# montyhall/bot7

Hardware: AMD Instinct MI355X
Metric: EI candidates scored/sec at N=2048,d=32 (higher is better)
Workload: dtype f64

## Files before the change

### bot7_amd/build.py

```python
import concurrent.futures
import os
import subprocess
import sys

HERE = os.path.dirname(os.path.abspath(__file__))
ROOT = os.path.dirname(HERE)
CSRC = os.path.join(HERE, "csrc")
BUILD = os.path.join(HERE, "_build")
OUT = os.path.join(HERE, "libbot7hip.so")
SOURCES = ["context.hip", "grid_api.hip", "gp_api.hip", "nominate.hip", "blr_api.hip", "sobol.hip", "covar.hip", "potrf.hip", "potrf_persist.hip", "posterior.hip", "score.hip", "extras.hip", "comm.hip", "group.hip", "blr_small.hip", "gp_small.hip", "kpost_small.hip", "batch.hip", "mes.hip", "rff.hip", "slice.hip", "refine.hip", "kg.hip"]
DIAG_ONLY_SOURCES = ["nll_small.hip"]
DIAG_OUT = os.path.join(ROOT, "tools", "_build", "libbot7hip_diag.so")
HEADERS = [os.path.join(CSRC, "b7_internal.h"), os.path.join(CSRC, "gemm_f64.h"), os.path.join(CSRC, "potrf_diag.h"), os.path.join(CSRC, "comm_rccl.h"), os.path.join(CSRC, "ksx_exp.h"), os.path.join(CSRC, "exp_table.h"), os.path.join(CSRC, "mes_math.h"), os.path.join(CSRC, "counter_rng.h"), os.path.join(CSRC, "gp_small_body.h"),
           os.path.join(ROOT, "include", "bot7hip.h")]
HIPCC = os.environ.get("HIPCC", "/opt/rocm/bin/hipcc")
FLAGS = ["-O3", "-std=c++17", "-fPIC", "--offload-arch=gfx950", "-fno-fast-math", "-Wall",
         "-I" + os.path.join(ROOT, "include"), "-I" + CSRC, "-I/opt/rocm/include"]


def _stale(target, deps):
    if not os.path.exists(target):
        return True
    t = os.path.getmtime(target)
    return any(os.path.getmtime(d) > t for d in deps)


EXTRA_FLAGS = {"covar.hip": ["-mllvm", "-amdgpu-mfma-vgpr-form"], "batch.hip": ["-mllvm", "-amdgpu-mfma-vgpr-form"],
               "rff.hip": ["-mllvm", "-amdgpu-mfma-vgpr-form"],
               "kg.hip": ["-mllvm", "-amdgpu-mfma-vgpr-form"],
               "slice.hip": ["-mllvm", "-disable-machine-licm"]}


def _compile(src, diag=False):
    obj = os.path.join(BUILD, ("diag_" if diag else "") + src.replace(".hip", ".o"))
    path = os.path.join(CSRC, src)
    if _stale(obj, [path] + HEADERS + [os.path.abspath(__file__)]):
        subprocess.check_call([HIPCC] + FLAGS + EXTRA_FLAGS.get(src, []) + (["-DB7_DIAG"] if diag else []) + ["-c", path, "-o", obj])
        return obj, True
    return obj, False


def _mentions_diag(src):
    return "B7_DIAG" in open(os.path.join(CSRC, src)).read()


def build_diag(verbose=False):
    build()
    os.makedirs(os.path.dirname(DIAG_OUT), exist_ok=True)
    todo = [s for s in SOURCES if _mentions_diag(s)] + DIAG_ONLY_SOURCES
    with concurrent.futures.ThreadPoolExecutor(max_workers=min(8, len(todo))) as ex:
        res = dict(zip(todo, ex.map(lambda s: _compile(s, True), todo)))
    objs = [res[s][0] if s in res else os.path.join(BUILD, s.replace(".hip", ".o")) for s in SOURCES + DIAG_ONLY_SOURCES]
    if any(ch for _, ch in res.values()) or _stale(DIAG_OUT, objs):
        subprocess.check_call([HIPCC, "-shared", "-fPIC", "--offload-arch=gfx950", "-o", DIAG_OUT] + objs +
                              ["-ldl", "-Wl,-rpath,/opt/rocm/lib", "-Wl,--no-undefined", "-Wl,-Bsymbolic"])
        if verbose:
            print("built", DIAG_OUT)
    return DIAG_OUT


def posterior_isa():
    out = os.path.join(BUILD, "posterior.s")
    path = os.path.join(CSRC, "posterior.hip")
    if _stale(out, [path] + HEADERS + [os.path.abspath(__file__)]):
        subprocess.check_call([HIPCC] + [f for f in FLAGS if f != "-fPIC"] + ["-S", "--cuda-device-only", "-Wno-unused-command-line-argument",
                                                                            path, "-o", out])
    return out


def check_agpr_discipline():
    import re
    text = open(posterior_isa()).read()
    found = {}
    for m in re.finditer(r"^(_ZN\S*post_kernel_w4(?:ILi(\d)E|tILi\d+ELi\d+E)\S*):[^\n]*\n(.*?)\n\s*s_endpgm", text, flags=re.S | re.M):
        nj = int(m.group(2)) if m.group(2) else 16
        ntiles = 32 if nj == 16 else 8 * nj
        in_asm, stats, bad = False, {"mfma": 0, "mfma_from_zero": 0, "acc_reads": 0, "scratch": 0}, []
        for line in m.group(3).split("\n"):
            code = line.split(";")[0]
            if "ASMSTART" in line:
                in_asm = True
                continue
            if "ASMEND" in line:
                in_asm = False
                continue
            if in_asm:
                stats["mfma"] += "v_mfma_f64_16x16x4_f64" in code
                stats["mfma_from_zero"] += bool(re.search(r"v_mfma_f64_16x16x4_f64 a\[[^\]]*\], v\[[^\]]*\], v\[[^\]]*\], 0\s*$", code))
                stats["acc_reads"] += "v_accvgpr_read_b32" in code
            else:
                if re.search(r"(?<![A-Za-z0-9_.])a(\[|\d)", code):
                    bad.append(line.strip())
                stats["scratch"] += "scratch_" in code
        if bad or stats["scratch"] or stats["mfma_from_zero"] != ntiles or stats["acc_reads"] != 8 * ntiles:
            raise RuntimeError("post_kernel_w4<%d>: AGPR discipline broken: %r, compiler-generated AGPR uses: %r"
                               % (nj, stats, bad[:5]))
        found[nj] = stats
    if not {2, 4} <= set(found):
        raise RuntimeError("post_kernel_w4<2> and <4> expected in the ISA of posterior.hip, found %r" % sorted(found))
    return found


def build_post_probe():
    src = os.path.join(ROOT, "tools", "post_probe.hip")
    out = os.path.join(ROOT, "tools", "_build", "post_probe")
    os.makedirs(os.path.dirname(out), exist_ok=True)
    if _stale(out, [src, os.path.join(ROOT, "tools", "post_kernel_w8.h"), os.path.join(CSRC, "posterior.hip")] + HEADERS):
        subprocess.check_call([HIPCC, "--offload-arch=gfx950", "-O3", "-std=c++17", "-fno-fast-math", "-Wno-unused-value",
                               "-DB7_POST_NO_LAUNCHERS", "-I" + os.path.join(ROOT, "include"), "-I" + CSRC,
                               "-I/opt/rocm/include", "-o", out, src, "-Wl,-rpath,/opt/rocm/lib"])
    return out


def build(force=False, verbose=False):
    os.makedirs(BUILD, exist_ok=True)
    if force:
        for f in os.listdir(BUILD):
            os.remove(os.path.join(BUILD, f))
    with concurrent.futures.ThreadPoolExecutor(max_workers=min(8, len(SOURCES) + 2)) as ex:
        isa = ex.submit(check_agpr_discipline)
        probe = ex.submit(build_post_probe)
        results = list(ex.map(_compile, SOURCES))
        isa.result()
        probe.result()
    objs = [o for o, _ in results]
    if any(changed for _, changed in results) or _stale(OUT, objs):
        subprocess.check_call([HIPCC, "-shared", "-fPIC", "--offload-arch=gfx950", "-o", OUT] + objs +
                              ["-ldl", "-Wl,-rpath,/opt/rocm/lib", "-Wl,--no-undefined", "-Wl,-Bsymbolic"])
        if verbose:
            print("built", OUT)
    return OUT


if __name__ == "__main__":
    build(force="--force" in sys.argv, verbose=True)
    if "--diag" in sys.argv:
        build_diag(verbose=True)
```

### bot7_amd/csrc/posterior.hip

```cpp
#include "b7_internal.h"
#include <utility>

#ifdef B7_POST_STAMPS
__device__ unsigned long long b7_post_stamps[4 * 4096];
extern "C" int b7dbg_post_stamps(unsigned long long *out, int nblocks) {
  return (int)hipMemcpyFromSymbol(out, HIP_SYMBOL(b7_post_stamps), sizeof(unsigned long long) * 4 * nblocks);
}
#endif

typedef double d2_t __attribute__((ext_vector_type(2)));

struct PostBatch {
  int64_t sLinv = 0, sks = 0, svar = 0;
  const double *base = nullptr, *var_add = nullptr;
};

namespace w4 {
constexpr int BM = 128, BK = 16, LD = BK + 1, A_DBL = BM * LD;

#define B7_W4_ACC_REGS \
  "a0", "a1", "a2", "a3", "a4", "a5", "a6", "a7", "a8", "a9", "a10", "a11", "a12", "a13", "a14", "a15", \
  "a16", "a17", "a18", "a19", "a20", "a21", "a22", "a23", "a24", "a25", "a26", "a27", "a28", "a29", "a30", \
  "a31", "a32", "a33", "a34", "a35", "a36", "a37", "a38", "a39", "a40", "a41", "a42", "a43", "a44", "a45", \
  "a46", "a47", "a48", "a49", "a50", "a51", "a52", "a53", "a54", "a55", "a56", "a57", "a58", "a59", "a60", \
  "a61", "a62", "a63", "a64", "a65", "a66", "a67", "a68", "a69", "a70", "a71", "a72", "a73", "a74", "a75", \
  "a76", "a77", "a78", "a79", "a80", "a81", "a82", "a83", "a84", "a85", "a86", "a87", "a88", "a89", "a90", \
  "a91", "a92", "a93", "a94", "a95", "a96", "a97", "a98", "a99", "a100", "a101", "a102", "a103", "a104", \
  "a105", "a106", "a107", "a108", "a109", "a110", "a111", "a112", "a113", "a114", "a115", "a116", "a117", \
  "a118", "a119", "a120", "a121", "a122", "a123", "a124", "a125", "a126", "a127", "a128", "a129", "a130", \
  "a131", "a132", "a133", "a134", "a135", "a136", "a137", "a138", "a139", "a140", "a141", "a142", "a143", \
  "a144", "a145", "a146", "a147", "a148", "a149", "a150", "a151", "a152", "a153", "a154", "a155", "a156", \
  "a157", "a158", "a159", "a160", "a161", "a162", "a163", "a164", "a165", "a166", "a167", "a168", "a169", \
  "a170", "a171", "a172", "a173", "a174", "a175", "a176", "a177", "a178", "a179", "a180", "a181", "a182", \
  "a183", "a184", "a185", "a186", "a187", "a188", "a189", "a190", "a191", "a192", "a193", "a194", "a195", \
  "a196", "a197", "a198", "a199", "a200", "a201", "a202", "a203", "a204", "a205", "a206", "a207", "a208", \
  "a209", "a210", "a211", "a212", "a213", "a214", "a215", "a216", "a217", "a218", "a219", "a220", "a221", \
  "a222", "a223", "a224", "a225", "a226", "a227", "a228", "a229", "a230", "a231", "a232", "a233", "a234", \
  "a235", "a236", "a237", "a238", "a239", "a240", "a241", "a242", "a243", "a244", "a245", "a246", "a247", \
  "a248", "a249", "a250", "a251", "a252", "a253", "a254", "a255"

template <int NJ, int I, int J, bool ZERO>
__device__ __forceinline__ void mfma_tile(double a, double b) {
  constexpr int lo = 8 * (NJ * I + J);
  if constexpr (ZERO)
    asm volatile("v_mfma_f64_16x16x4_f64 a[%2:%3], %0, %1, 0" ::"v"(a), "v"(b), "n"(lo), "n"(lo + 7) : B7_W4_ACC_REGS);
  else
    asm volatile("v_mfma_f64_16x16x4_f64 a[%2:%3], %0, %1, a[%2:%3]" ::"v"(a), "v"(b), "n"(lo), "n"(lo + 7)
                 : B7_W4_ACC_REGS);
}

template <int NJ, int I, int J>
__device__ __forceinline__ void read_tile(double (&v)[4]) {
  constexpr int lo = 8 * (NJ * I + J);
  unsigned w[8];
  asm volatile(
      "v_accvgpr_read_b32 %0, a[%8]\n\tv_accvgpr_read_b32 %1, a[%9]\n\tv_accvgpr_read_b32 %2, a[%10]\n\t"
      "v_accvgpr_read_b32 %3, a[%11]\n\tv_accvgpr_read_b32 %4, a[%12]\n\tv_accvgpr_read_b32 %5, a[%13]\n\t"
      "v_accvgpr_read_b32 %6, a[%14]\n\tv_accvgpr_read_b32 %7, a[%15]"
      : "=v"(w[0]), "=v"(w[1]), "=v"(w[2]), "=v"(w[3]), "=v"(w[4]), "=v"(w[5]), "=v"(w[6]), "=v"(w[7])
      : "n"(lo), "n"(lo + 1), "n"(lo + 2), "n"(lo + 3), "n"(lo + 4), "n"(lo + 5), "n"(lo + 6), "n"(lo + 7));
#pragma unroll
  for (int r = 0; r < 4; ++r) v[r] = __hiloint2double((int)w[2 * r + 1], (int)w[2 * r]);
}

template <int NJ>
struct Frags {
  double a[2][8], b[2][NJ];
};
template <int NJ>
struct Stage {
  d2_t c[4 + 2 * NJ];
};
struct Cursor {
  int t, kb, ntiles;
  __device__ __forceinline__ void advance() {
    if (kb + 1 < (t + 1) * (BM / BK)) {
      ++kb;
    } else if (t + 1 < ntiles) {
      ++t;
      kb = 0;
    }
  }
};

template <int N, class F, int... Is>
__device__ __forceinline__ void static_for_impl(F &&f, std::integer_sequence<int, Is...>) {
  (f(std::integral_constant<int, Is>{}), ...);
}
template <int N, class F>
__device__ __forceinline__ void static_for(F &&f) {
  static_for_impl<N>(f, std::make_integer_sequence<int, N>{});
}

template <int NJ, int P, int S0>
__device__ __forceinline__ void read_pair(Frags<NJ> &f, const double *__restrict__ sa, const double *__restrict__ sb) {
  if constexpr (P < NJ) {
    f.b[0][P] = sb[P * 16 * LD + 4 * S0];
    f.b[1][P] = sb[P * 16 * LD + 4 * S0 + 4];
  } else {
    f.a[0][P - NJ] = sa[(P - NJ) * 16 * LD + 4 * S0];
    f.a[1][P - NJ] = sa[(P - NJ) * 16 * LD + 4 * S0 + 4];
  }
}

template <int NJ, int C>
__device__ __forceinline__ void load_chunk(Stage<NJ> &g, const double *__restrict__ qa, const double *__restrict__ qb,
                                           int64_t lda) {
  if constexpr (C < 4)
    g.c[C] = *reinterpret_cast<const d2_t *>(qa + (int64_t)(32 * C) * lda);
  else
    g.c[C] = *reinterpret_cast<const d2_t *>(qb + (int64_t)(32 * (C - 4)) * lda);
}
template <int NJ, int C>
__device__ __forceinline__ void store_chunk(const Stage<NJ> &g, double *__restrict__ w) {
  constexpr int o = C < 4 ? 32 * C * LD : A_DBL + 32 * (C - 4) * LD;
  w[o] = g.c[C][0];
  w[o + 1] = g.c[C][1];
}

template <int NJ, int FIRST, bool ZERO>
__device__ __forceinline__ void stage(Frags<NJ> &f0, Frags<NJ> &f1, Stage<NJ> &g, double *__restrict__ cur,
                                      double *__restrict__ nxt, int fa, int fb, int wofs, const double *__restrict__ pa,
                                      const double *__restrict__ pb, int64_t lda, Cursor &ld) {
  constexpr int NI = 8 - FIRST, NM = 2 * NJ * NI, NP = 8 + NJ, NC = 4 + 2 * NJ, NS = NP + 2 * NC;
  const double *qa = pa + ((int64_t)ld.t * BM) * lda + ld.kb * BK, *qb = pb + ld.kb * BK;
  ld.advance();
  constexpr int K1 = (NS + NM - 1) / NM + 1, K2 = (NP + NM - 1) / NM + 1;
  static_for<NM>([&](auto m_) {
    constexpr int m = decltype(m_)::value, ks = m / (NJ * NI), i = FIRST + (m % (NJ * NI)) / NJ, j = m % NJ;
    mfma_tile<NJ, i, j, ZERO && ks == 0>(f0.a[ks][i], f0.b[ks][j]);
    static_for<K1>([&](auto k_) {
      constexpr int sidx = m * NS / NM + decltype(k_)::value;
      if constexpr (sidx < (m + 1) * NS / NM) {
        if constexpr (sidx < NP) {
          if constexpr (sidx < NJ || sidx - NJ >= FIRST) read_pair<NJ, sidx, 2>(f1, cur + fa, cur + fb);
        } else if constexpr (sidx < NP + NC) {
          store_chunk<NJ, sidx - NP>(g, nxt + wofs);
        } else {
          load_chunk<NJ, sidx - NP - NC>(g, qa, qb, lda);
        }
      }
    });
  });
  __builtin_amdgcn_s_waitcnt(0xC07F);
  __builtin_amdgcn_s_barrier();
  static_for<NM>([&](auto m_) {
    constexpr int m = decltype(m_)::value, ks = m / (NJ * NI), i = FIRST + (m % (NJ * NI)) / NJ, j = m % NJ;
    mfma_tile<NJ, i, j, false>(f1.a[ks][i], f1.b[ks][j]);
    static_for<K2>([&](auto k_) {
      constexpr int sidx = m * NP / NM + decltype(k_)::value;
      if constexpr (sidx < (m + 1) * NP / NM) read_pair<NJ, sidx, 0>(f0, nxt + fa, nxt + fb);
    });
  });
}

template <int NJ>
__global__ void __launch_bounds__(256)
    post_kernel_w4(const double *__restrict__ Linv, const double *__restrict__ ks, int Npad, int64_t row0, int64_t Mtotal,
                   double base, double sgn, double var_add, int clamp, double var_min, double *__restrict__ var,
                   PostBatch bat) {
  constexpr int BN = 64 * NJ, STAGE_DBL = (BM + BN) * LD, NC = 4 + 2 * NJ, NP = 8 + NJ;
  extern __shared__ __align__(16) double sm[];
  if (bat.base) {
    const int64_t y = blockIdx.y;
    Linv += y * bat.sLinv;
    ks += y * bat.sks;
    var += y * bat.svar;
    base = bat.base[y];
    if (bat.var_add) var_add = bat.var_add[y];
  }
  const int lane = threadIdx.x & 63, wave = __builtin_amdgcn_readfirstlane(threadIdx.x >> 6);
#ifdef B7_POST_STAMPS
  const unsigned long long st0 = __builtin_amdgcn_s_memtime(), sr0 = __builtin_amdgcn_s_memrealtime();
  __builtin_amdgcn_s_waitcnt(0xC07F);
#endif
  const int64_t lda = Npad;
  const int r0 = threadIdx.x >> 3, kc = threadIdx.x & 7;
  const double *pa = Linv + (int64_t)r0 * lda + 2 * kc;
  const double *pb = ks + ((int64_t)blockIdx.x * BN + r0) * lda + 2 * kc;
  const int wofs = r0 * LD + 2 * kc;
  const int fa = (lane & 15) * LD + (lane >> 4);
  const int fb = A_DBL + (wave * 16 * NJ + (lane & 15)) * LD + (lane >> 4);

  const int ntiles = Npad / BM;
  Cursor ld{0, 0, ntiles};
  Stage<NJ> g;
  Frags<NJ> f0, f1;
  double *const b0 = sm, *const b1 = sm + STAGE_DBL;
  static_for<NC>([&](auto c_) { load_chunk<NJ, decltype(c_)::value>(g, pa, pb, lda); });
  ld.advance();
  static_for<NC>([&](auto c_) { store_chunk<NJ, decltype(c_)::value>(g, b0 + wofs); });
  {
    const double *qa = pa + ((int64_t)ld.t * BM) * lda + ld.kb * BK, *qb = pb + ld.kb * BK;
    static_for<NC>([&](auto c_) { load_chunk<NJ, decltype(c_)::value>(g, qa, qb, lda); });
    ld.advance();
  }
  __builtin_amdgcn_s_waitcnt(0xC07F);
  __builtin_amdgcn_s_barrier();
  static_for<NP>([&](auto p_) { read_pair<NJ, decltype(p_)::value, 0>(f0, b0 + fa, b0 + fb); });

  double colss[2][NJ] = {};
#define B7_STAGE(F, Z, CUR, NXT) stage<NJ, F, Z>(f0, f1, g, CUR, NXT, fa, fb, wofs, pa, pb, lda, ld)
  for (int t = 0; t < ntiles; ++t) {
    B7_STAGE(0, true, b0, b1);
    if (t > 0) {
      for (int p = 0; p < 4 * t - 1; ++p) {
        B7_STAGE(0, false, b1, b0);
        B7_STAGE(0, false, b0, b1);
      }
      B7_STAGE(0, false, b1, b0);
      B7_STAGE(0, false, b0, b1);
    }
    B7_STAGE(1, false, b1, b0);
    B7_STAGE(2, false, b0, b1);
    B7_STAGE(3, false, b1, b0);
    B7_STAGE(4, false, b0, b1);
    B7_STAGE(5, false, b1, b0);
    B7_STAGE(6, false, b0, b1);
    B7_STAGE(7, false, b1, b0);
    asm volatile("s_nop 15\n\ts_nop 15\n\ts_nop 15" ::: "memory");
    static_for<2 * NJ>([&](auto hj_) {
      constexpr int h = decltype(hj_)::value / NJ, j = decltype(hj_)::value % NJ;
      double s = 0.0;
      static_for<4>([&](auto i_) {
        double v[4];
        read_tile<NJ, 4 * h + decltype(i_)::value, j>(v);
#pragma unroll
        for (int r = 0; r < 4; ++r) s = __builtin_fma(v[r], v[r], s);
      });
      colss[h][j] += s;
    });
  }
#undef B7_STAGE

#pragma unroll
  for (int j = 0; j < NJ; ++j) {
    double v0 = colss[0][j], v1 = colss[1][j];
    v0 += __shfl_xor(v0, 16);
    v0 += __shfl_xor(v0, 32);
    v1 += __shfl_xor(v1, 16);
    v1 += __shfl_xor(v1, 32);
    const int64_t gidx = row0 + (int64_t)blockIdx.x * BN + wave * 16 * NJ + j * 16 + lane;
    if (lane < 16 && gidx < Mtotal) {
      double ss = v0;
      ss += v1;
      double v = (base + sgn * ss) + var_add;
      if (clamp) v = (v < var_min) ? var_min : v;
      var[gidx] = v;
    }
  }
#ifdef B7_POST_STAMPS
  if (threadIdx.x == 0 && blockIdx.x < 4096) {
    const unsigned long long st1 = __builtin_amdgcn_s_memtime(), sr1 = __builtin_amdgcn_s_memrealtime();
    __builtin_amdgcn_s_waitcnt(0xC07F);
    unsigned long long *o = b7_post_stamps + 4 * blockIdx.x;
    o[0] = st0, o[1] = sr0, o[2] = st1, o[3] = sr1;
  }
#endif
}

template <int NJ>
constexpr int lds_bytes() { return 2 * (BM + 64 * NJ) * LD * 8; }

template <int NJ, int NR>
struct Tall {
  static constexpr int BMT = 16 * NR, BN = 64 * NJ, A_DBLT = BMT * LD, STAGE_DBL = (BMT + BN) * LD;
  static constexpr int NCA = BMT / 32, NC = NCA + 2 * NJ, NP = NR + NJ;
  static constexpr int LDS_BYTES = 2 * STAGE_DBL * 8;
  static_assert(NJ * NR == 32, "32 accumulator tiles per wave");

  struct Set {
    double a[NR], b[NJ];
  };
  struct Data {
    d2_t c[NC];
  };
  struct Cursor {
    int t, kb, ntiles;
    __device__ __forceinline__ void advance() {
      if (kb + 1 < (t + 1) * (BMT / BK)) {
        ++kb;
      } else if (t + 1 < ntiles) {
        ++t;
        kb = 0;
      }
    }
  };

  template <int P, int S>
  static __device__ __forceinline__ void read_one(Set &f, const double *__restrict__ sa, const double *__restrict__ sb) {
    if constexpr (P < NJ)
      f.b[P] = sb[P * 16 * LD + 4 * S];
    else
      f.a[P - NJ] = sa[(P - NJ) * 16 * LD + 4 * S];
  }
  template <int C>
  static __device__ __forceinline__ void load_chunk(Data &g, const double *__restrict__ qa, const double *__restrict__ qb,
                                                    int64_t lda) {
    if constexpr (C < NCA)
      g.c[C] = *reinterpret_cast<const d2_t *>(qa + (int64_t)(32 * C) * lda);
    else
      g.c[C] = *reinterpret_cast<const d2_t *>(qb + (int64_t)(32 * (C - NCA)) * lda);
  }
  template <int C>
  static __device__ __forceinline__ void store_chunk(const Data &g, double *__restrict__ w) {
    constexpr int o = C < NCA ? 32 * C * LD : A_DBLT + 32 * (C - NCA) * LD;
    w[o] = g.c[C][0];
    w[o + 1] = g.c[C][1];
  }

  template <int FIRST, bool ZERO, int NSIDE, class Side>
  static __device__ __forceinline__ void kstep(const Set &use, Side &&side) {
    constexpr int NI = NR - FIRST, NM = NJ * NI;
    constexpr int KMAX = (NSIDE + NM - 1) / NM + 1;
    static_for<NM>([&](auto m_) {
      constexpr int m = decltype(m_)::value, i = FIRST + m / NJ, j = m % NJ;
      mfma_tile<NJ, i, j, ZERO>(use.a[i], use.b[j]);
      static_for<KMAX>([&](auto k_) {
        constexpr int sidx = m * NSIDE / NM + decltype(k_)::value;
        if constexpr (sidx < (m + 1) * NSIDE / NM) side(std::integral_constant<int, sidx>{});
      });
    });
  }

  template <int FIRST, int NEXT_FIRST, bool ZERO>
  static __device__ __forceinline__ void stage(Set &s0, Set &s1, Data &g, double *__restrict__ cur, double *__restrict__ nxt,
                                               int fa, int fb, int wofs, const double *__restrict__ pa,
                                               const double *__restrict__ pb, int64_t lda, Cursor &ld) {
    constexpr int H = NC / 2;
    const double *qa = pa + ((int64_t)ld.t * BMT) * lda + ld.kb * BK, *qb = pb + ld.kb * BK;
    ld.advance();
    kstep<FIRST, ZERO, NP + H>(s0, [&](auto s_) {
      constexpr int x = decltype(s_)::value;
      if constexpr (x < NP) {
        if constexpr (x < NJ || x - NJ >= FIRST) read_one<x, 1>(s1, cur + fa, cur + fb);
      } else {
        store_chunk<x - NP>(g, nxt + wofs);
      }
    });
    kstep<FIRST, false, NP + NC - H>(s1, [&](auto s_) {
      constexpr int x = decltype(s_)::value;
      if constexpr (x < NP) {
        if constexpr (x < NJ || x - NJ >= FIRST) read_one<x, 2>(s0, cur + fa, cur + fb);
      } else {
        store_chunk<H + x - NP>(g, nxt + wofs);
      }
    });
    kstep<FIRST, false, NP + NC>(s0, [&](auto s_) {
      constexpr int x = decltype(s_)::value;
      if constexpr (x < NP) {
        if constexpr (x < NJ || x - NJ >= FIRST) read_one<x, 3>(s1, cur + fa, cur + fb);
      } else {
        load_chunk<x - NP>(g, qa, qb, lda);
      }
    });
    __builtin_amdgcn_s_waitcnt(0xC07F);
    __builtin_amdgcn_s_barrier();
    kstep<FIRST, false, NP>(s1, [&](auto s_) {
      constexpr int x = decltype(s_)::value;
      if constexpr (x < NJ || x - NJ >= NEXT_FIRST) read_one<x, 0>(s0, nxt + fa, nxt + fb);
    });
  }
};

template <int NJ, int NR>
__global__ void __launch_bounds__(256)
    post_kernel_w4t(const double *__restrict__ Linv, const double *__restrict__ ks, int Npad, int64_t row0, int64_t Mtotal,
                    double base, double sgn, double var_add, int clamp, double var_min, double *__restrict__ var,
                    PostBatch bat) {
  using T = Tall<NJ, NR>;
  constexpr int BMT = T::BMT, BN = T::BN, NC = T::NC, NP = T::NP;
  extern __shared__ __align__(16) double sm[];
  if (bat.base) {
    const int64_t y = blockIdx.y;
    Linv += y * bat.sLinv;
    ks += y * bat.sks;
    var += y * bat.svar;
    base = bat.base[y];
    if (bat.var_add) var_add = bat.var_add[y];
  }
  const int lane = threadIdx.x & 63, wave = __builtin_amdgcn_readfirstlane(threadIdx.x >> 6);
#ifdef B7_POST_STAMPS
  const unsigned long long st0 = __builtin_amdgcn_s_memtime(), sr0 = __builtin_amdgcn_s_memrealtime();
  __builtin_amdgcn_s_waitcnt(0xC07F);
#endif
  const int64_t lda = Npad;
  const int r0 = threadIdx.x >> 3, kc = threadIdx.x & 7;
  const double *pa = Linv + (int64_t)r0 * lda + 2 * kc;
  const double *pb = ks + ((int64_t)blockIdx.x * BN + r0) * lda + 2 * kc;
  const int wofs = r0 * LD + 2 * kc;
  const int fa = (lane & 15) * LD + (lane >> 4);
  const int fb = T::A_DBLT + (wave * 16 * NJ + (lane & 15)) * LD + (lane >> 4);

  const int ntiles = Npad / BMT;
  typename T::Cursor ld{0, 0, ntiles};
  typename T::Data g;
  typename T::Set s0, s1;
  double *const b0 = sm, *const b1 = sm + T::STAGE_DBL;
  static_for<NC>([&](auto c_) { T::template load_chunk<decltype(c_)::value>(g, pa, pb, lda); });
  ld.advance();
  static_for<NC>([&](auto c_) { T::template store_chunk<decltype(c_)::value>(g, b0 + wofs); });
  {
    const double *qa = pa + ((int64_t)ld.t * BMT) * lda + ld.kb * BK, *qb = pb + ld.kb * BK;
    static_for<NC>([&](auto c_) { T::template load_chunk<decltype(c_)::value>(g, qa, qb, lda); });
    ld.advance();
  }
  __builtin_amdgcn_s_waitcnt(0xC07F);
  __builtin_amdgcn_s_barrier();
  static_for<NP>([&](auto p_) { T::template read_one<decltype(p_)::value, 0>(s0, b0 + fa, b0 + fb); });

  double colss[2][NJ] = {};
#define B7_STAGE(F, NF, Z, CUR, NXT) T::template stage<F, NF, Z>(s0, s1, g, CUR, NXT, fa, fb, wofs, pa, pb, lda, ld)
  for (int t = 0; t < ntiles; ++t) {
    B7_STAGE(0, 0, true, b0, b1);
    if (t > 0) {
      for (int p = 0; p < (NR / 2) * t - 1; ++p) {
        B7_STAGE(0, 0, false, b1, b0);
        B7_STAGE(0, 0, false, b0, b1);
      }
      B7_STAGE(0, 0, false, b1, b0);
      B7_STAGE(0, 1, false, b0, b1);
    }
    static_for<NR - 1>([&](auto q_) {
      constexpr int Q = decltype(q_)::value + 1;
      if constexpr (Q % 2 == 1)
        B7_STAGE(Q, (Q + 1) % NR, false, b1, b0);
      else
        B7_STAGE(Q, (Q + 1) % NR, false, b0, b1);
    });
    asm volatile("s_nop 15\n\ts_nop 15\n\ts_nop 15" ::: "memory");
    static_for<(NR / 4) * NJ>([&](auto qj_) {
      constexpr int q = decltype(qj_)::value / NJ, j = decltype(qj_)::value % NJ;
      double s = 0.0;
      static_for<4>([&](auto i_) {
        double v[4];
        read_tile<NJ, 4 * q + decltype(i_)::value, j>(v);
#pragma unroll
        for (int r = 0; r < 4; ++r) s = __builtin_fma(v[r], v[r], s);
      });
      colss[q & 1][j] += s;
    });
  }
#undef B7_STAGE

#pragma unroll
  for (int j = 0; j < NJ; ++j) {
    double v0 = colss[0][j], v1 = colss[1][j];
    v0 += __shfl_xor(v0, 16);
    v0 += __shfl_xor(v0, 32);
    v1 += __shfl_xor(v1, 16);
    v1 += __shfl_xor(v1, 32);
    const int64_t gidx = row0 + (int64_t)blockIdx.x * BN + wave * 16 * NJ + j * 16 + lane;
    if (lane < 16 && gidx < Mtotal) {
      double ss = v0;
      ss += v1;
      double v = (base + sgn * ss) + var_add;
      if (clamp) v = (v < var_min) ? var_min : v;
      var[gidx] = v;
    }
  }
#ifdef B7_POST_STAMPS
  if (threadIdx.x == 0 && blockIdx.x < 4096) {
    const unsigned long long st1 = __builtin_amdgcn_s_memtime(), sr1 = __builtin_amdgcn_s_memrealtime();
    __builtin_amdgcn_s_waitcnt(0xC07F);
    unsigned long long *o = b7_post_stamps + 4 * blockIdx.x;
    o[0] = st0, o[1] = sr0, o[2] = st1, o[3] = sr1;
  }
#endif
}
}

namespace small64 {
typedef double d4_t __attribute__((ext_vector_type(4)));
constexpr int NB = 64, LLD = NB + 2, BN = 64;
constexpr int LDS_BYTES = BN * LLD * 8;

__global__ void __launch_bounds__(256)
    post_small_kernel(const double *__restrict__ Linv, const double *__restrict__ ks, int64_t row0, int64_t Mtotal, int ntiles,
                      double base, double sgn, double var_add, int clamp, double var_min, double *__restrict__ var, PostBatch bat) {
  extern __shared__ __align__(16) double sm[];
  if (bat.base) {
    const int64_t y = blockIdx.y;
    Linv += y * bat.sLinv;
    ks += y * bat.sks;
    var += y * bat.svar;
    base = bat.base[y];
    if (bat.var_add) var_add = bat.var_add[y];
  }
  double *Ks = sm;
  const int tid = threadIdx.x, lane = tid & 63, wave = tid >> 6, lr = lane & 15, lq = lane >> 4;
  d2_t pv[BN / 8];
  auto fetch = [&](int tile) {
    const double *kt = ks + ((int64_t)tile * BN) * NB;
#pragma unroll
    for (int i = 0; i < BN / 8; ++i) {
      const int e = tid + 256 * i;
      pv[i] = *reinterpret_cast<const d2_t *>(kt + (int64_t)(e >> 5) * NB + 2 * (e & 31));
    }
  };
  int tile = blockIdx.x;
  if (tile < ntiles) fetch(tile);
  double af[40];
#pragma unroll
  for (int I = 0; I < 4; ++I)
#pragma unroll
    for (int k4 = 0; k4 < 4 * (I + 1); ++k4) af[2 * I * (I + 1) + k4] = Linv[(int64_t)(I * 16 + lr) * NB + 4 * k4 + lq];
#pragma unroll
  for (int g = 0; g < 4; ++g)
    asm volatile("" : "+v"(af[10 * g]), "+v"(af[10 * g + 1]), "+v"(af[10 * g + 2]), "+v"(af[10 * g + 3]), "+v"(af[10 * g + 4]),
                      "+v"(af[10 * g + 5]), "+v"(af[10 * g + 6]), "+v"(af[10 * g + 7]), "+v"(af[10 * g + 8]), "+v"(af[10 * g + 9]));
  for (; tile < ntiles; tile += gridDim.x) {
#pragma unroll
    for (int i = 0; i < BN / 8; ++i) {
      const int e = tid + 256 * i, r = e >> 5, c2 = 2 * (e & 31);
      Ks[r * LLD + c2] = pv[i][0];
      Ks[r * LLD + c2 + 1] = pv[i][1];
    }
    __syncthreads();
    if (tile + (int)gridDim.x < ntiles) fetch(tile + gridDim.x);
    __builtin_amdgcn_sched_barrier(0);
    constexpr int NJ = BN / 64;
    double ss[NJ];
#pragma unroll
    for (int j = 0; j < NJ; ++j) {
      const double *bp = Ks + (wave * 16 * NJ + j * 16 + lr) * LLD + lq;
      double bf[16];
#pragma unroll
      for (int k4 = 0; k4 < 16; ++k4) bf[k4] = bp[4 * k4];
      double s = 0.0;
#pragma unroll
      for (int I = 0; I < 4; ++I) {
        d4_t c = {0.0, 0.0, 0.0, 0.0};
#ifdef B7_PS_ABLATE
        c = __builtin_amdgcn_mfma_f64_16x16x4f64(af[2 * I * (I + 1)], bf[I], c, 0, 0, 0);
#else
#pragma unroll
        for (int k4 = 0; k4 < 4 * (I + 1); ++k4) c = __builtin_amdgcn_mfma_f64_16x16x4f64(af[2 * I * (I + 1) + k4], bf[k4], c, 0, 0, 0);
#endif
#pragma unroll
        for (int r = 0; r < 4; ++r) s = __builtin_fma(c[r], c[r], s);
      }
      ss[j] = s;
    }
#pragma unroll
    for (int j = 0; j < NJ; ++j) {
      double v = ss[j];
      v += __shfl_xor(v, 16);
      v += __shfl_xor(v, 32);
      const int64_t gidx = row0 + (int64_t)tile * BN + wave * 16 * NJ + j * 16 + lr;
      if (lane < 16 && gidx < Mtotal) {
        double o = (base + sgn * v) + var_add;
        if (clamp) o = (o < var_min) ? var_min : o;
        var[gidx] = o;
      }
    }
    __syncthreads();
  }
}
}

#ifndef B7_POST_NO_LAUNCHERS
namespace {
struct PostArgs {
  const double *Linv, *ks;
  double *var;
  double base, sgn, var_add;
  int S;
  PostBatch pb;
};

template <int NJ>
int launch_post_w4(b7_ctx *c, const PostArgs &a, int64_t row0, int64_t rows, int64_t Mtotal) {
  constexpr int lds = w4::lds_bytes<NJ>();
  B7_HIP(c, hipFuncSetAttribute(reinterpret_cast<const void *>(w4::post_kernel_w4<NJ>),
                                hipFuncAttributeMaxDynamicSharedMemorySize, lds));
  hipLaunchKernelGGL(w4::post_kernel_w4<NJ>, dim3((unsigned)(rows / (64 * NJ)), a.S), dim3(256), lds, c->stream, a.Linv, a.ks,
                     c->Npad, row0, Mtotal, a.base, a.sgn, a.var_add, c->opts.var_clamp, c->opts.var_min, a.var, a.pb);
  B7_HIP(c, hipGetLastError());
  return B7_OK;
}

template <int NJ, int NR>
int launch_post_tall(b7_ctx *c, const PostArgs &a, int64_t row0, int64_t rows, int64_t Mtotal) {
  using T = w4::Tall<NJ, NR>;
  auto kern = w4::post_kernel_w4t<NJ, NR>;
  B7_HIP(c, hipFuncSetAttribute(reinterpret_cast<const void *>(kern), hipFuncAttributeMaxDynamicSharedMemorySize,
                                T::LDS_BYTES));
  hipLaunchKernelGGL(kern, dim3((unsigned)(rows / T::BN), a.S), dim3(256), T::LDS_BYTES, c->stream, a.Linv, a.ks, c->Npad, row0,
                     Mtotal, a.base, a.sgn, a.var_add, c->opts.var_clamp, c->opts.var_min, a.var, a.pb);
  B7_HIP(c, hipGetLastError());
  return B7_OK;
}

int launch_post_small(b7_ctx *c, const PostArgs &a, int64_t row0, int64_t rows, int64_t Mtotal) {
  B7_HIP(c, hipFuncSetAttribute(reinterpret_cast<const void *>(small64::post_small_kernel), hipFuncAttributeMaxDynamicSharedMemorySize,
                                small64::LDS_BYTES));
  const int ntiles = (int)(rows / small64::BN), S = a.S > 0 ? a.S : 1;
  int gx = (2 * c->cus + S - 1) / S;
  if (gx > ntiles) gx = ntiles;
  if (gx < 1) gx = 1;
  hipLaunchKernelGGL(small64::post_small_kernel, dim3((unsigned)gx, S), dim3(256), small64::LDS_BYTES, c->stream, a.Linv, a.ks, row0,
                     Mtotal, ntiles, a.base, a.sgn, a.var_add, c->opts.var_clamp, c->opts.var_min, a.var, a.pb);
  B7_HIP(c, hipGetLastError());
  return B7_OK;
}

int dispatch_post(b7_ctx *c, const PostArgs &a, int64_t row0, int64_t rows, int64_t Mtotal) {
  if (rows % B7_MROWS) return b7_fail(c, B7_ERR_INVALID, "post: rows %lld not a multiple of %d", (long long)rows, B7_MROWS);
  if (c->Npad == 64) return launch_post_small(c, a, row0, rows, Mtotal);
  const bool large = rows / 256 * a.S >= c->cus;
  if (c->Npad % 256 == 0 && large) return launch_post_tall<2, 16>(c, a, row0, rows, Mtotal);
  if (!large) return launch_post_w4<2>(c, a, row0, rows, Mtotal);
  return launch_post_w4<4>(c, a, row0, rows, Mtotal);
}
}

int launch_post(b7_ctx *c, const FitSet &f, const double *ks, int64_t row0, int64_t rows, int64_t Mtotal, double *var) {
  PhaseScope ps(c, "post");
  const bool blr = c->model_kind == 1;
  PostArgs a{f.Linv, ks, var, blr ? 0.0 : f.amp, blr ? 1.0 : -1.0, blr ? f.noise : (c->opts.var_with_noise ? f.noise : 0.0), 1,
             PostBatch{}};
  return dispatch_post(c, a, row0, rows, Mtotal);
}

int launch_post_batch(b7_ctx *c, const FitSet &f, const double *ks, int64_t sks, int64_t rows, int64_t Mtotal, double *var,
                      int64_t svar) {
  PhaseScope ps(c, "post");
  PostArgs a{f.Linv, ks, var, 0.0, -1.0, 0.0, f.S, PostBatch{}};
  a.pb.sLinv = FitSet::s_Linv(c->Npad, c->dpad);
  a.pb.sks = sks;
  a.pb.svar = svar;
  a.pb.base = f.amp_dev;
  a.pb.var_add = c->opts.var_with_noise ? f.noise_dev : nullptr;
  return dispatch_post(c, a, 0, rows, Mtotal);
}

int launch_post_heads(b7_ctx *c, int S, const double *Linv, const double *feat, int64_t rows, int64_t Mtotal, double *var, int64_t svar,
                      const double *zero_dev, const double *invbeta_dev) {
  PhaseScope ps(c, "post");
  PostArgs a{Linv, feat, var, 0.0, 1.0, 0.0, S, PostBatch{}};
  a.pb.sLinv = FitSet::s_Linv(c->Npad, c->dpad);
  a.pb.sks = 0;
  a.pb.svar = svar;
  a.pb.base = zero_dev;
  a.pb.var_add = invbeta_dev;
  return dispatch_post(c, a, 0, rows, Mtotal);
}
#endif
```

Before: 16.14 million.

## Stream posterior tiles via direct global-to-LDS DMA into a triple-buffered swizzled ring

Replaces the register-staged global load plus LDS store path in the tall posterior kernel with global_load_lds_dwordx4 instructions that write 1 KiB pieces straight into LDS through m0. The double buffer becomes a three-stage ring with an XOR-swizzled row layout, and fragment addresses rotate across buffers. The aim is to free VGPRs and issue slots spent on staging stores and to keep two tiles in flight ahead of the MFMA work. It adds explicit m0 handling, a vmcnt-based wait, more LDS use, and a build check that the compiler emits no stray m0 uses.

```diff
diff --git a/bot7_amd/build.py b/bot7_amd/build.py
--- a/bot7_amd/build.py
+++ b/bot7_amd/build.py
@@ -11,7 +11,7 @@
 SOURCES = ["context.hip", "grid_api.hip", "gp_api.hip", "nominate.hip", "blr_api.hip", "sobol.hip", "covar.hip", "potrf.hip", "potrf_persist.hip", "posterior.hip", "score.hip", "extras.hip", "comm.hip", "group.hip", "blr_small.hip", "gp_small.hip", "kpost_small.hip", "batch.hip", "mes.hip", "rff.hip", "slice.hip", "refine.hip", "kg.hip"]
 DIAG_ONLY_SOURCES = ["nll_small.hip"]
 DIAG_OUT = os.path.join(ROOT, "tools", "_build", "libbot7hip_diag.so")
-HEADERS = [os.path.join(CSRC, "b7_internal.h"), os.path.join(CSRC, "gemm_f64.h"), os.path.join(CSRC, "potrf_diag.h"), os.path.join(CSRC, "comm_rccl.h"), os.path.join(CSRC, "ksx_exp.h"), os.path.join(CSRC, "exp_table.h"), os.path.join(CSRC, "mes_math.h"), os.path.join(CSRC, "counter_rng.h"), os.path.join(CSRC, "gp_small_body.h"),
+HEADERS = [os.path.join(CSRC, "b7_internal.h"), os.path.join(CSRC, "gemm_f64.h"), os.path.join(CSRC, "potrf_diag.h"), os.path.join(CSRC, "comm_rccl.h"), os.path.join(CSRC, "ksx_exp.h"), os.path.join(CSRC, "exp_table.h"), os.path.join(CSRC, "mes_math.h"), os.path.join(CSRC, "counter_rng.h"), os.path.join(CSRC, "gp_small_body.h"), os.path.join(CSRC, "post_ring_layout.h"),
            os.path.join(ROOT, "include", "bot7hip.h")]
 HIPCC = os.environ.get("HIPCC", "/opt/rocm/bin/hipcc")
 FLAGS = ["-O3", "-std=c++17", "-fPIC", "--offload-arch=gfx950", "-fno-fast-math", "-Wall",
@@ -91,6 +91,8 @@
             else:
                 if re.search(r"(?<![A-Za-z0-9_.])a(\[|\d)", code):
                     bad.append(line.strip())
+                if nj == 16 and re.search(r"\bm0\b", code):
+                    bad.append(line.strip())
                 stats["scratch"] += "scratch_" in code
         if bad or stats["scratch"] or stats["mfma_from_zero"] != ntiles or stats["acc_reads"] != 8 * ntiles:
             raise RuntimeError("post_kernel_w4<%d>: AGPR discipline broken: %r, compiler-generated AGPR uses: %r"
diff --git a/bot7_amd/csrc/post_ring_layout.h b/bot7_amd/csrc/post_ring_layout.h
--- /dev/null
+++ b/bot7_amd/csrc/post_ring_layout.h
@@ -0,0 +1,22 @@
+#pragma once
+
+namespace post_ring {
+constexpr int CHUNK_BYTES = 16, ROW_BYTES = 128, PIECE_BYTES = 1024, PIECE_ROWS = PIECE_BYTES / ROW_BYTES, WAVES = 4;
+
+struct Chunk {
+  int row, chunk;
+};
+
+constexpr int swz(int row) { return (row >> 1) & 7; }
+
+constexpr int slot_byte(int row, int chunk) { return row * ROW_BYTES + (chunk ^ swz(row)) * CHUNK_BYTES; }
+
+constexpr Chunk dma_src(int piece, int lane) {
+  const int row = piece * PIECE_ROWS + (lane >> 3);
+  return Chunk{row, (lane & 7) ^ swz(row)};
+}
+
+constexpr int piece_of(int wave, int i) { return WAVES * i + wave; }
+
+constexpr int frag_byte(int row, int k) { return slot_byte(row, k >> 1) + (k & 1) * 8; }
+}
diff --git a/bot7_amd/csrc/posterior.hip b/bot7_amd/csrc/posterior.hip
--- a/bot7_amd/csrc/posterior.hip
+++ b/bot7_amd/csrc/posterior.hip
@@ -1,4 +1,5 @@
 #include "b7_internal.h"
+#include "post_ring_layout.h"
 #include <utility>
 
 #ifdef B7_POST_STAMPS
@@ -264,16 +265,37 @@
 
 template <int NJ, int NR>
 struct Tall {
-  static constexpr int BMT = 16 * NR, BN = 64 * NJ, A_DBLT = BMT * LD, STAGE_DBL = (BMT + BN) * LD;
-  static constexpr int NCA = BMT / 32, NC = NCA + 2 * NJ, NP = NR + NJ;
-  static constexpr int LDS_BYTES = 2 * STAGE_DBL * 8;
+  static constexpr int BMT = 16 * NR, BN = 64 * NJ, ROWS = BMT + BN;
+  static constexpr int STAGE_BYTES = ROWS * post_ring::ROW_BYTES, NBUF = 3;
+  static constexpr int ND = ROWS / post_ring::PIECE_ROWS / post_ring::WAVES;
+  static constexpr int NDA = BMT / post_ring::PIECE_ROWS / post_ring::WAVES;
+  static constexpr int NP = NR + NJ;
+  static constexpr int LDS_BYTES = NBUF * STAGE_BYTES;
   static_assert(NJ * NR == 32, "32 accumulator tiles per wave");
+  static_assert(ND == 12 && ND % 3 == 0, "vmcnt(12) below is ND; a third of the pieces per k-step");
+  static_assert(LDS_BYTES <= 160 * 1024, "three stage images in 160 KiB");
 
   struct Set {
     double a[NR], b[NJ];
   };
-  struct Data {
-    d2_t c[NC];
+  typedef __attribute__((address_space(3))) double lds_double;
+  struct Lane {
+    int fa[NBUF][4], fb[NBUF][4];
+    unsigned src, dst[NBUF];
+    __device__ __forceinline__ void rotate1() {
+#pragma unroll
+      for (int s = 0; s < 4; ++s) {
+        const int a = fa[0][s], b = fb[0][s];
+        fa[0][s] = fa[1][s], fa[1][s] = fa[2][s], fa[2][s] = a;
+        fb[0][s] = fb[1][s], fb[1][s] = fb[2][s], fb[2][s] = b;
+      }
+      const unsigned d = dst[0];
+      dst[0] = dst[1], dst[1] = dst[2], dst[2] = d;
+    }
+    __device__ __forceinline__ void rotate(int k) {
+      if (k >= 1) rotate1();
+      if (k >= 2) rotate1();
+    }
   };
   struct Cursor {
     int t, kb, ntiles;
@@ -287,78 +309,66 @@
     }
   };
 
-  template <int P, int S>
-  static __device__ __forceinline__ void read_one(Set &f, const double *__restrict__ sa, const double *__restrict__ sb) {
+  template <int P, int S, int B>
+  static __device__ __forceinline__ void read_one(Set &f, const Lane &ln) {
+    constexpr int strip = (P < NJ ? P : P - NJ) * 16 * post_ring::ROW_BYTES;
     if constexpr (P < NJ)
-      f.b[P] = sb[P * 16 * LD + 4 * S];
+      f.b[P] = *reinterpret_cast<const lds_double *>((uintptr_t)(unsigned)(ln.fb[B][S] + strip));
     else
-      f.a[P - NJ] = sa[(P - NJ) * 16 * LD + 4 * S];
+      f.a[P - NJ] = *reinterpret_cast<const lds_double *>((uintptr_t)(unsigned)(ln.fa[B][S] + strip));
   }
   template <int C>
-  static __device__ __forceinline__ void load_chunk(Data &g, const double *__restrict__ qa, const double *__restrict__ qb,
-                                                    int64_t lda) {
-    if constexpr (C < NCA)
-      g.c[C] = *reinterpret_cast<const d2_t *>(qa + (int64_t)(32 * C) * lda);
-    else
-      g.c[C] = *reinterpret_cast<const d2_t *>(qb + (int64_t)(32 * (C - NCA)) * lda);
-  }
-  template <int C>
-  static __device__ __forceinline__ void store_chunk(const Data &g, double *__restrict__ w) {
-    constexpr int o = C < NCA ? 32 * C * LD : A_DBLT + 32 * (C - NCA) * LD;
-    w[o] = g.c[C][0];
-    w[o + 1] = g.c[C][1];
-  }
-
-  template <int FIRST, bool ZERO, int NSIDE, class Side>
+  static __device__ __forceinline__ void dma_piece(const char *__restrict__ ga, const char *__restrict__ gb, int64_t step,
+                                                   unsigned src, unsigned dst) {
+    const char *g = C < NDA ? ga + C * step : gb + (C - NDA) * step;
+    const unsigned m0 = dst + C * post_ring::WAVES * post_ring::PIECE_BYTES;
+    asm volatile("s_mov_b32 m0, %0\n\ts_nop 0\n\tglobal_load_lds_dwordx4 %1, %2" ::"s"(m0), "v"(src), "s"(g) : "memory");
+  }
+
+  template <int FIRST, bool ZERO, int NSIDE, int TAIL, class Side>
   static __device__ __forceinline__ void kstep(const Set &use, Side &&side) {
-    constexpr int NI = NR - FIRST, NM = NJ * NI;
-    constexpr int KMAX = (NSIDE + NM - 1) / NM + 1;
+    constexpr int NI = NR - FIRST, NM = NJ * NI, NMS = NM > 2 * TAIL ? NM - TAIL : NM;
+    constexpr int KMAX = (NSIDE + NMS - 1) / NMS + 1;
     static_for<NM>([&](auto m_) {
       constexpr int m = decltype(m_)::value, i = FIRST + m / NJ, j = m % NJ;
       mfma_tile<NJ, i, j, ZERO>(use.a[i], use.b[j]);
-      static_for<KMAX>([&](auto k_) {
-        constexpr int sidx = m * NSIDE / NM + decltype(k_)::value;
-        if constexpr (sidx < (m + 1) * NSIDE / NM) side(std::integral_constant<int, sidx>{});
-      });
+      if constexpr (m < NMS)
+        static_for<KMAX>([&](auto k_) {
+          constexpr int sidx = m * NSIDE / NMS + decltype(k_)::value;
+          if constexpr (sidx < (m + 1) * NSIDE / NMS) side(std::integral_constant<int, sidx>{});
+        });
     });
   }
-
-  template <int FIRST, int NEXT_FIRST, bool ZERO>
-  static __device__ __forceinline__ void stage(Set &s0, Set &s1, Data &g, double *__restrict__ cur, double *__restrict__ nxt,
-                                               int fa, int fb, int wofs, const double *__restrict__ pa,
-                                               const double *__restrict__ pb, int64_t lda, Cursor &ld) {
-    constexpr int H = NC / 2;
-    const double *qa = pa + ((int64_t)ld.t * BMT) * lda + ld.kb * BK, *qb = pb + ld.kb * BK;
+  static constexpr int H = ND / 3, NS = NP + H;
+  static constexpr int dma_before(int x) {
+    int n = 0;
+    for (int d = 0; d < H; ++d) n += (d + 1) * NS / (H + 1) < x;
+    return n;
+  }
+  static constexpr bool is_dma(int x) { return dma_before(x + 1) > dma_before(x); }
+
+  template <int FIRST, int NEXT_FIRST, bool ZERO, int POS>
+  static __device__ __forceinline__ void stage(Set &s0, Set &s1, const Lane &ln,
+                                               const char *__restrict__ pa, const char *__restrict__ pb, int64_t lda, Cursor &ld) {
+    constexpr int CUR = POS % NBUF, NXT = (POS + 1) % NBUF, DST = (POS + 2) % NBUF;
+    const int64_t step = 32 * lda * 8;
+    const char *ga = pa + (((int64_t)ld.t * BMT) * lda + ld.kb * BK) * 8, *gb = pb + (int64_t)(ld.kb * BK) * 8;
     ld.advance();
-    kstep<FIRST, ZERO, NP + H>(s0, [&](auto s_) {
+    auto sides = [&](auto ks_, Set &into, auto x_) {
+      constexpr int ks = decltype(ks_)::value, x = decltype(x_)::value, r = x - dma_before(x);
+      if constexpr (is_dma(x))
+        dma_piece<H * ks + dma_before(x)>(ga, gb, step, ln.src, ln.dst[DST]);
+      else if constexpr (r < NJ || r - NJ >= FIRST)
+        read_one<r, ks + 1, CUR>(into, ln);
+    };
+    kstep<FIRST, ZERO, NS, 0>(s0, [&](auto x_) { sides(std::integral_constant<int, 0>{}, s1, x_); });
+    kstep<FIRST, false, NS, 0>(s1, [&](auto x_) { sides(std::integral_constant<int, 1>{}, s0, x_); });
+    kstep<FIRST, false, NS, 3>(s0, [&](auto x_) { sides(std::integral_constant<int, 2>{}, s1, x_); });
+    asm volatile("s_waitcnt vmcnt(12) lgkmcnt(0)" ::: "memory");
+    __builtin_amdgcn_s_barrier();
+    kstep<FIRST, false, NP, 0>(s1, [&](auto s_) {
       constexpr int x = decltype(s_)::value;
-      if constexpr (x < NP) {
-        if constexpr (x < NJ || x - NJ >= FIRST) read_one<x, 1>(s1, cur + fa, cur + fb);
-      } else {
-        store_chunk<x - NP>(g, nxt + wofs);
-      }
-    });
-    kstep<FIRST, false, NP + NC - H>(s1, [&](auto s_) {
-      constexpr int x = decltype(s_)::value;
-      if constexpr (x < NP) {
-        if constexpr (x < NJ || x - NJ >= FIRST) read_one<x, 2>(s0, cur + fa, cur + fb);
-      } else {
-        store_chunk<H + x - NP>(g, nxt + wofs);
-      }
-    });
-    kstep<FIRST, false, NP + NC>(s0, [&](auto s_) {
-      constexpr int x = decltype(s_)::value;
-      if constexpr (x < NP) {
-        if constexpr (x < NJ || x - NJ >= FIRST) read_one<x, 3>(s1, cur + fa, cur + fb);
-      } else {
-        load_chunk<x - NP>(g, qa, qb, lda);
-      }
-    });
-    __builtin_amdgcn_s_waitcnt(0xC07F);
-    __builtin_amdgcn_s_barrier();
-    kstep<FIRST, false, NP>(s1, [&](auto s_) {
-      constexpr int x = decltype(s_)::value;
-      if constexpr (x < NJ || x - NJ >= NEXT_FIRST) read_one<x, 0>(s0, nxt + fa, nxt + fb);
+      if constexpr (x < NJ || x - NJ >= NEXT_FIRST) read_one<x, 0, NXT>(s0, ln);
     });
   }
 };
@@ -369,7 +379,7 @@
                     double base, double sgn, double var_add, int clamp, double var_min, double *__restrict__ var,
                     PostBatch bat) {
   using T = Tall<NJ, NR>;
-  constexpr int BMT = T::BMT, BN = T::BN, NC = T::NC, NP = T::NP;
+  constexpr int BMT = T::BMT, BN = T::BN, NP = T::NP;
   extern __shared__ __align__(16) double sm[];
   if (bat.base) {
     const int64_t y = blockIdx.y;
@@ -385,49 +395,61 @@
   __builtin_amdgcn_s_waitcnt(0xC07F);
 #endif
   const int64_t lda = Npad;
-  const int r0 = threadIdx.x >> 3, kc = threadIdx.x & 7;
-  const double *pa = Linv + (int64_t)r0 * lda + 2 * kc;
-  const double *pb = ks + ((int64_t)blockIdx.x * BN + r0) * lda + 2 * kc;
-  const int wofs = r0 * LD + 2 * kc;
-  const int fa = (lane & 15) * LD + (lane >> 4);
-  const int fb = T::A_DBLT + (wave * 16 * NJ + (lane & 15)) * LD + (lane >> 4);
+  const char *pa = reinterpret_cast<const char *>(Linv + (int64_t)(post_ring::PIECE_ROWS * wave) * lda);
+  const char *pb = reinterpret_cast<const char *>(ks + ((int64_t)blockIdx.x * BN + post_ring::PIECE_ROWS * wave) * lda);
+  typename T::Lane ln;
+  {
+    const post_ring::Chunk c = post_ring::dma_src(wave, lane);
+    ln.src = (unsigned)(((c.row - post_ring::PIECE_ROWS * wave) * Npad + 2 * c.chunk) * 8);
+  }
+  const unsigned lds0 = (unsigned)(uintptr_t)(__attribute__((address_space(3))) void *)sm;
+#pragma unroll
+  for (int b = 0; b < T::NBUF; ++b) {
+#pragma unroll
+    for (int s = 0; s < 4; ++s) {
+      ln.fa[b][s] = lds0 + b * T::STAGE_BYTES + post_ring::frag_byte(lane & 15, 4 * s + (lane >> 4));
+      ln.fb[b][s] = ln.fa[b][s] + (BMT + wave * 16 * NJ) * post_ring::ROW_BYTES;
+      asm volatile("" : "+v"(ln.fa[b][s]), "+v"(ln.fb[b][s]));
+    }
+    ln.dst[b] = lds0 + b * T::STAGE_BYTES + wave * post_ring::PIECE_BYTES;
+  }
 
   const int ntiles = Npad / BMT;
   typename T::Cursor ld{0, 0, ntiles};
-  typename T::Data g;
   typename T::Set s0, s1;
-  double *const b0 = sm, *const b1 = sm + T::STAGE_DBL;
-  static_for<NC>([&](auto c_) { T::template load_chunk<decltype(c_)::value>(g, pa, pb, lda); });
-  ld.advance();
-  static_for<NC>([&](auto c_) { T::template store_chunk<decltype(c_)::value>(g, b0 + wofs); });
   {
-    const double *qa = pa + ((int64_t)ld.t * BMT) * lda + ld.kb * BK, *qb = pb + ld.kb * BK;
-    static_for<NC>([&](auto c_) { T::template load_chunk<decltype(c_)::value>(g, qa, qb, lda); });
+    const int64_t step = 32 * lda * 8;
+    static_for<T::ND>([&](auto c_) { T::template dma_piece<decltype(c_)::value>(pa, pb, step, ln.src, ln.dst[0]); });
     ld.advance();
-  }
-  __builtin_amdgcn_s_waitcnt(0xC07F);
+    const char *ga = pa + (((int64_t)ld.t * BMT) * lda + ld.kb * BK) * 8, *gb = pb + (int64_t)(ld.kb * BK) * 8;
+    static_for<T::ND>([&](auto c_) { T::template dma_piece<decltype(c_)::value>(ga, gb, step, ln.src, ln.dst[1]); });
+    ld.advance();
+  }
+  asm volatile("s_waitcnt vmcnt(12)" ::: "memory");
   __builtin_amdgcn_s_barrier();
-  static_for<NP>([&](auto p_) { T::template read_one<decltype(p_)::value, 0>(s0, b0 + fa, b0 + fb); });
+  static_for<NP>([&](auto p_) { T::template read_one<decltype(p_)::value, 0, 0>(s0, ln); });
 
   double colss[2][NJ] = {};
-#define B7_STAGE(F, NF, Z, CUR, NXT) T::template stage<F, NF, Z>(s0, s1, g, CUR, NXT, fa, fb, wofs, pa, pb, lda, ld)
+#define B7_STAGE(F, NF, Z, POS) T::template stage<F, NF, Z, POS>(s0, s1, ln, pa, pb, lda, ld)
   for (int t = 0; t < ntiles; ++t) {
-    B7_STAGE(0, 0, true, b0, b1);
+    B7_STAGE(0, 0, true, 0);
     if (t > 0) {
-      for (int p = 0; p < (NR / 2) * t - 1; ++p) {
-        B7_STAGE(0, 0, false, b1, b0);
-        B7_STAGE(0, 0, false, b0, b1);
+      const int n = NR * t - 1;
+      for (int p = 0; p < n / 3; ++p) {
+        B7_STAGE(0, 0, false, 1);
+        B7_STAGE(0, 0, false, 2);
+        B7_STAGE(0, 0, false, 0);
       }
-      B7_STAGE(0, 0, false, b1, b0);
-      B7_STAGE(0, 1, false, b0, b1);
+      if (n % 3 >= 1) B7_STAGE(0, 0, false, 1);
+      if (n % 3 == 2) B7_STAGE(0, 0, false, 2);
+      ln.rotate((n + 1) % 3);
+      B7_STAGE(0, 1, false, 0);
     }
     static_for<NR - 1>([&](auto q_) {
       constexpr int Q = decltype(q_)::value + 1;
-      if constexpr (Q % 2 == 1)
-        B7_STAGE(Q, (Q + 1) % NR, false, b1, b0);
-      else
-        B7_STAGE(Q, (Q + 1) % NR, false, b0, b1);
+      B7_STAGE(Q, (Q + 1) % NR, false, Q % 3);
     });
+    ln.rotate(NR % 3);
     asm volatile("s_nop 15\n\ts_nop 15\n\ts_nop 15" ::: "memory");
     static_for<(NR / 4) * NJ>([&](auto qj_) {
       constexpr int q = decltype(qj_)::value / NJ, j = decltype(qj_)::value % NJ;
@@ -442,6 +464,7 @@
     });
   }
 #undef B7_STAGE
+  asm volatile("s_waitcnt vmcnt(0)" ::: "memory");
 
 #pragma unroll
   for (int j = 0; j < NJ; ++j) {
```

Result: faster. 16.47 million, median of 6 (+2.1%).
